# rrahn/libspm

Measured on AMD Instinct MI355X. Metric: Gbases/s scanned, Myers k<=3 |P|=100, higher is better.
Workload: dtype u32

## Files before the change

### libspm_amd/csrc/filter.hpp

```cpp
#pragma once

#include "brute.hpp"
#include "common.hpp"
#include "filter_shared.hpp"
#include "pack.hpp"
#include "hd.hpp"

namespace spm_hip
{

struct survivor
{
    uint32_t key;
    uint32_t t_lo, t_hi;
    uint32_t pad;
};
constexpr uint32_t kSurvInvalid = 0xFFFFFFFFu;

struct band_rec
{
    uint32_t slot;
    uint32_t val;
    uint32_t seg;
    uint32_t band;
// ... 785 lines not shown
                prev[4 * u + 3] = cur[u].z;
            }
            filter_words<S, NWD, HV, 4, true, KM>(P, w, prev, nv, base0 + ch * 4096, lane, lds, idx_mask);
        }
        sp += n_waves;
    }
    surv_close(P, cand_chunk_of(P, lds), lane);
}

struct verify_params
{
    const uint8_t *text;
    uint64_t text_alloc;
    uint64_t ctx_begin;
    uint64_t scan_begin;
    uint64_t scan_end;
    uint64_t pos_offset;
    const band_rec *bands;
    const unsigned long long *counters;
    uint32_t band_counter;
    uint32_t preselected;
    uint64_t band_cap;
    ulonglong2 *band_tab;
    uint32_t table_mask, band_bits;
    uint32_t runs;
    const uint8_t *surplus;
    uint32_t Bw;
    uint32_t overlap;
    uint32_t max_m;
    const uint32_t *peq32;
    uint32_t sigma;
    uint32_t nw_table;
    uint32_t max_k;
    const int32_t *m;
    const int32_t *k;
    uint32_t report_begin;
    uint32_t max_span;
    uint32_t wave_text;
    unsigned long long *seen;
    uint32_t seen_mask;
    spm_hit *hits;
    unsigned long long *hit_counter;
    uint64_t hit_cap;
    unsigned long long *overflow;
    const uint64_t *seg_offsets;
    uint64_t n_segments;
    const uint32_t *seg_owned;
};

struct resolve_params
{
    const survivor *surv;
    unsigned long long *counters;
    uint64_t surv_cap;
    const pass_entry *passes;
    const uint4 *entries;
    uint32_t key_len;
    uint32_t flank_check;
    uint32_t pieces_check;
    const uint8_t *text;
    uint64_t text_alloc;
    const uint8_t *needle_ranks;
    const uint32_t *needle_offsets;
    const uint16_t *seed_q;
    const int32_t *m, *k;
    uint64_t hay_begin, hay_end;
    const uint64_t *seg_offsets;
    uint64_t n_segments;
    uint32_t Bw, overlap, max_m;
    uint32_t band_bits;
    ulonglong2 *band_tab;
    uint32_t table_mask;
    band_rec *bands;
    uint64_t band_cap;
    const uint32_t *needle_pk;
    const uint32_t *pk_offsets;
    uint32_t exact_hits;
    uint32_t report_begin;
    uint64_t scan_begin, scan_end;
    uint64_t pos_offset;
    const uint32_t *seg_owned;
    unsigned long long *seen;
    uint32_t seen_mask;
    spm_hit *hits;
    unsigned long long *hit_counter, *overflow;
    uint64_t hit_cap;
    uint32_t *table_poison;
};

__device__ __forceinline__ unsigned long long band_value(unsigned long long stored, bool counting)
{
    return counting ? (unsigned long long)(uint32_t)(stored + 1ull) : ~stored;
}
__device__ __forceinline__ void band_release(ulonglong2 *tab, uint32_t slot)
{
    tab[slot] = make_ulonglong2(kBandEmpty, ~0ull);
}

__device__ __forceinline__ uint4 load_bytes16(const uint8_t *p)
{
    uint4 v;
    __builtin_memcpy(&v, p, 16);
    return v;
}

__device__ __forceinline__ uint4 load_bytes16_guarded(const uint8_t *base, uint64_t idx, uint64_t limit)
{
    if (idx + 16 <= limit)
        return load_bytes16(base + idx);
    uint32_t w[4] = {0xFFFFFFFFu, 0xFFFFFFFFu, 0xFFFFFFFFu, 0xFFFFFFFFu};
    for (int b = 0; b < 16; ++b)
        if (idx + b < limit)
            w[b >> 2] = (w[b >> 2] & ~(0xFFu << (8 * (b & 3)))) | ((uint32_t)base[idx + b] << (8 * (b & 3)));
    return make_uint4(w[0], w[1], w[2], w[3]);
}

__device__ __forceinline__ uint32_t diff16(const uint4 a, const uint4 b, uint32_t n)
{
    const uint32_t d[4] = {a.x ^ b.x, a.y ^ b.y, a.z ^ b.z, a.w ^ b.w};
    uint32_t r = 0;
#pragma unroll
    for (uint32_t i = 0; i < 4; ++i) {
        const uint32_t have = n > 4 * i ? n - 4 * i : 0;
        const uint32_t mask = have >= 4 ? 0xFFFFFFFFu : (have == 0 ? 0u : (1u << (8 * have)) - 1);
        r |= d[i] & mask;
    }
    return r;
}

__device__ __forceinline__ bool seed_intact(const resolve_params &P, uint64_t t, uint32_t val, uint32_t r, uint32_t q_whole,
                                            int64_t hay_b, int64_t hay_e)
{
    if (!P.needle_ranks)
        return true;
    const uint32_t pat = val >> 11, x = val & 0x7FF;
    struct
    {
        uint32_t q;
    } sp{q_whole ? q_whole : P.seed_q[pat]};
    const uint32_t o = x - r;
    const int64_t ts = (int64_t)t - (int64_t)r;
    if (ts < hay_b || ts + (int64_t)sp.q > hay_e)
        return false;
    const uint8_t *nd = P.needle_ranks + P.needle_offsets[pat] + o;
    for (uint32_t i = 0; i < sp.q; i += 16) {
        const uint32_t n = sp.q - i < 16 ? sp.q - i : 16;
        if (diff16(load_bytes16_guarded(P.text, (uint64_t)ts + i, P.text_alloc), load_bytes16(nd + i), n))
            return false;
    }
    return true;
}

constexpr uint32_t kPieceRoundsShift = 21, kPieceMissingShift = 28;

__device__ __forceinline__ bool pieces_apply(const resolve_params &P, uint64_t t, uint32_t val, uint32_t m, uint32_t k, int64_t hay_b,
                                             int64_t hay_e)
{
    if (!P.pieces_check || k == 0 || k > 7 || m < 32)
        return false;
    const int64_t d = (int64_t)t - (int64_t)(val & 0x7FF);
    return d - (int64_t)k >= hay_b && d + (int64_t)(m + k) <= hay_e;
}

__device__ __forceinline__ uint32_t pieces_visit(const resolve_params &P, uint64_t t, uint32_t val, uint32_t &rng, uint32_t m, uint32_t k)
{
    const uint32_t pat = val >> 11, x = val & 0x7FF;
    const uint32_t n_rounds = m >> 4;
    uint32_t done = (rng >> kPieceRoundsShift) & 0x7F, missing = (rng >> kPieceMissingShift) & 7;
    const bool ascending = 2 * x >= m;
    const uint32_t todo = n_rounds - done < 2 ? n_rounds - done : 2;
    const uint32_t r_lo = ascending ? done : n_rounds - done - todo;
    const uint32_t *pk = P.needle_pk + P.pk_offsets[pat] + r_lo;
    const uint32_t nw0 = pk[0], nw1 = todo == 2 ? pk[1] : 0;
    const uint64_t w0 = (uint64_t)((int64_t)t - (int64_t)x + (int64_t)(16 * r_lo) - (int64_t)k);
    const uint32_t c0 = pack16(load_bytes16_guarded(P.text, w0, P.text_alloc));
    const uint32_t c1 = pack16(load_bytes16_guarded(P.text, w0 + 16, P.text_alloc));
    const uint32_t c2 = todo == 2 ? pack16(load_bytes16_guarded(P.text, w0 + 32, P.text_alloc)) : 0;
#pragma unroll
    for (uint32_t rr = 0; rr < 2; ++rr) {
        if (rr < todo) {
            const uint32_t two = rr ? nw1 : nw0;
            const uint64_t win = rr ? ((uint64_t)c1 | ((uint64_t)c2 << 32)) : ((uint64_t)c0 | ((uint64_t)c1 << 32));
#pragma unroll
            for (uint32_t j = 0; j < 2; ++j) {
                const uint32_t piece = (two >> (16 * j)) & 0xFFFFu;
                bool found = false;
                for (uint32_t sh = 0; sh <= 2 * k; ++sh)
                    found = found || (((uint32_t)(win >> (2 * (8 * j + sh))) & 0xFFFFu) == piece);
                missing += found ? 0u : 1u;
            }
        }
    }
    if (missing > k)
        return 0;
    done += todo;
    if (done >= n_rounds)
        return 2;
    rng = (rng & ~((0x7Fu << kPieceRoundsShift) | (7u << kPieceMissingShift))) | (done << kPieceRoundsShift) |
          (missing << kPieceMissingShift);
    return 1;
}

struct text64
{
    uint64_t lo, hi;
    bool ok;
};

__device__ __forceinline__ uint32_t syms16(const text64 &W, uint32_t first)
{
    if (first >= 32)
        return (uint32_t)(W.hi >> (2 * (first - 32)));
    return (uint32_t)(W.lo >> (2 * first)) | (first ? (uint32_t)(W.hi << (2 * (32 - first)) ) : 0u);
}

__device__ __forceinline__ bool seed_sig_ok(const text64 &W, uint32_t sig, uint32_t r, uint32_t n, uint32_t H)
{
    if (n == 0)
        return true;
    const uint32_t rb = r < 16 ? r : 16;
    const uint32_t nl = rb < n ? rb : n;
    uint32_t got = nl ? syms16(W, 16 - rb) : 0u;
    if (nl < 16) {
        got &= (1u << (2 * nl)) - 1;
        got |= syms16(W, 16 + H) << (2 * nl);
    }
    const uint32_t mask = n >= 16 ? 0xFFFFFFFFu : ((1u << (2 * n)) - 1);
    return ((got ^ sig) & mask) == 0;
}

constexpr uint32_t kPairCap = 128;
struct pair_queue
{
// ... 128 lines not shown
                                                uint32_t pat, int64_t e)
{
    const unsigned long long key = ((unsigned long long)pat << 40) | (unsigned long long)e;
    uint32_t slot = (uint32_t)(mix64(key)) & seen_mask;
    for (uint32_t tries = 0; tries < 64; ++tries) {
        if (tries == 4 && __hip_atomic_load(overflow, __ATOMIC_RELAXED, __HIP_MEMORY_SCOPE_AGENT) != 0)
            return false;
        const unsigned long long old = atomicCAS(&seen[slot], ~0ull, key);
        if (old == ~0ull)
            return true;
        if (old == key)
            return false;
        slot = (slot + 1) & seen_mask;
    }
    atomicAdd(overflow, 1ull);
    return false;
}

struct resolve_wave
{
    pair_queue *Q;
    band_queue *B;
    uint32_t qn, bn;
    band_chunk C;
    uint32_t n_cand;
};

__device__ __forceinline__ void queue_sync()
{
    __builtin_amdgcn_fence(__ATOMIC_RELEASE, "wavefront");
    __builtin_amdgcn_wave_barrier();
}

__device__ __forceinline__ void check_pairs(const resolve_params &R, resolve_wave &S, uint32_t n, uint32_t lane)
{
    pair_queue &Q = *S.Q;
    band_queue &B = *S.B;
    S.qn -= n;
    const uint32_t first = S.qn;
    bool live = lane < n;
    uint64_t t = 0, seg = 0;
    uint32_t val = 0, rng = 0;
    int64_t sb = (int64_t)R.hay_begin, se = (int64_t)R.hay_end;
    if (live) {
        const uint32_t i = first + lane;
        t = ((uint64_t)Q.t_hi[i] << 32) | Q.t_lo[i];
        val = Q.val[i];
        rng = Q.rng[i];
        seg = Q.seg[i];
        if (R.seg_offsets) {
            sb = (int64_t)R.seg_offsets[seg];
            se = (int64_t)R.seg_offsets[seg + 1];
        }
    }
    queue_sync();
    bool through = live;
    const uint32_t pat = val >> 11;
    if (live && !(rng & kRngRun)) {
        if (!(rng & kSeedChecked)) {
            live = seed_intact(R, t, val, (rng >> 16) & 0x1F, (rng & kRngWhole) ? R.key_len + ((rng >> 5) & 0x1F) : 0u, sb, se);
            rng |= kSeedChecked;
        }
        through = live;
        if (live && R.pieces_check) {
            const uint32_t m = (uint32_t)R.m[pat], k = (uint32_t)R.k[pat];
            if (pieces_apply(R, t, val, m, k, sb, se)) {
                const uint32_t v = pieces_visit(R, t, val, rng, m, k);
                live = v != 0;
                through = v == 2;
            }
        }
    }
    {
        const bool back = live && !through;
        const uint64_t mm = __ballot(back);
        if (back) {
            const uint32_t q = S.qn + __popcll(mm & ((1ull << lane) - 1));
            Q.t_lo[q] = (uint32_t)t;
            Q.t_hi[q] = (uint32_t)(t >> 32);
            Q.val[q] = val;
            Q.rng[q] = rng;
            Q.seg[q] = (uint32_t)seg;
        }
        S.qn += __popcll(mm);
    }
    int64_t b_cur = 0, b_last = -1, d_lo = 0, d_hi = 0;
    if (R.exact_hits) {
        bool fresh = false;
        int64_t e = 0;
        if (live && through) {
            ++S.n_cand;
            e = (int64_t)t - (int64_t)(val & 0x7FF) + (int64_t)R.m[pat];
            int64_t own_b = (int64_t)R.scan_begin, own_e = (int64_t)R.scan_end;
            if (R.seg_offsets) {
                own_b = R.seg_owned ? sb + (int64_t)R.seg_owned[seg] : sb;
                own_e = se;
            }
            fresh = e >= own_b + 1 && e <= own_e && (!R.seen || seen_insert_raw(R.seen, R.seen_mask, R.overflow, pat, e));
        }
        const unsigned long long idx = wave_reserve_hits(R.hit_counter, fresh ? 1u : 0u);
        if (fresh && idx < R.hit_cap) {
            spm_hit h;
            h.pos = (R.report_begin ? (uint64_t)(e - (int64_t)R.m[pat]) : (uint64_t)e) + R.pos_offset;
            h.pattern = pat;
            h.score = 0;
            R.hits[idx] = h;
        }
        queue_sync();
        return;
    }
    if (live && through) {
        ++S.n_cand;
        d_hi = (int64_t)t - (int64_t)(val & 0x7FF) - sb + (int64_t)R.max_m;
        d_lo = d_hi - (int64_t)((rng & kRngRun) ? (rng & 0x7FF) : 0u);
        b_cur = d_lo / (int64_t)R.Bw;
        b_last = d_hi / (int64_t)R.Bw;
        if (R.overlap && b_cur > 0 && d_lo - b_cur * (int64_t)R.Bw <= (int64_t)R.k[pat])
            --b_cur;
        if ((uint64_t)b_last >> R.band_bits) {
            atomicAdd(&R.counters[kCntVoid], 1ull);
            b_last = b_cur - 1;
        }
    }
    for (;;) {
        const bool have = b_cur <= b_last;
        const uint64_t mm = __ballot(have);
        if (mm == 0)
            break;
        if (have) {
            const unsigned long long bkey =
                ((unsigned long long)pat << 43) | ((unsigned long long)seg << R.band_bits) | (unsigned long long)b_cur;
            const int64_t b0 = b_cur * (int64_t)R.Bw;
            const uint32_t o_lo = (uint32_t)(d_lo > b0 ? d_lo - b0 : 0);
            const uint32_t o_hi = (uint32_t)(d_hi < b0 + (int64_t)R.Bw - 1 ? d_hi - b0 : (int64_t)R.Bw - 1);
            const unsigned long long run = (o_hi - o_lo >= 63 ? ~0ull : ((1ull << (o_hi - o_lo + 1)) - 1)) << o_lo;
            const uint32_t q = S.bn + __popcll(mm & ((1ull << lane) - 1));
            B.key_lo[q] = (uint32_t)bkey;
            B.key_hi[q] = (uint32_t)(bkey >> 32);
            B.run_lo[q] = (uint32_t)run;
            B.run_hi[q] = (uint32_t)(run >> 32);
        }
        S.bn += __popcll(mm);
        queue_sync();
        if (S.bn >= 64) {
            S.bn -= 64;
            insert_bands(R, B, S.bn, 64, lane, S.C);
            queue_sync();
        }
        ++b_cur;
    }
    queue_sync();
}

__global__ __launch_bounds__(256) void resolve_kernel(const resolve_params R)
{
    __shared__ pair_queue pair_queues[4];
    __shared__ band_queue band_queues[4];
    unsigned long long n = R.counters[kCntSurvSlots];
    if (blockIdx.x == 0 && threadIdx.x == 0) {
        atomicAdd(&R.counters[kCntUnreadSurvSum], n);
        atomicMax(&R.counters[kCntUnreadSurvMax], n);
    }
    if (n > R.surv_cap)
        n = R.surv_cap;
    if (!R.exact_hits && __hip_atomic_load(R.table_poison, __ATOMIC_RELAXED, __HIP_MEMORY_SCOPE_AGENT) != 0) {
        if (blockIdx.x == 0 && threadIdx.x == 0)
            atomicAdd(&R.counters[kCntVoid], 1ull);
        return;
    }
    const uint32_t lane = threadIdx.x & 63;
    resolve_wave S;
    S.Q = &pair_queues[threadIdx.x >> 6];
    S.B = &band_queues[threadIdx.x >> 6];
    S.qn = 0;
    S.bn = 0;
    S.C.base = 0;
    S.C.used = 0;
    S.C.size = 0;
    S.C.draws = 0;
    S.n_cand = 0;
    pair_queue &Q = *S.Q;
    const uint64_t stride = (uint64_t)gridDim.x * blockDim.x;
    const uint64_t rounds = (n + stride - 1) / stride;
    for (uint64_t r = 0; r < rounds; ++r) {
        if ((r & 7u) == 7u &&
            __builtin_amdgcn_readfirstlane((uint32_t)(__hip_atomic_load(&R.counters[kCntVoid], __ATOMIC_RELAXED, __HIP_MEMORY_SCOPE_AGENT) != 0)))
            break;
        const uint64_t i = r * stride + (uint64_t)blockIdx.x * blockDim.x + threadIdx.x;
        bool probing = false;
        uint32_t key = 0;
        uint64_t t = 0, seg = 0;
        pass_entry T = R.passes[0];
        if (i < n) {
            const survivor sv = R.surv[i];
            if (sv.t_hi != kSurvInvalid) {
                probing = true;
                key = sv.key;
// ... 80 lines not shown
            OW.hi = ((uint64_t)(uint32_t)__shfl((int)(uint32_t)(W.hi >> 32), (int)owner) << 32) |
                    (uint32_t)__shfl((int)(uint32_t)W.hi, (int)owner);
            OW.ok = __shfl((int)W.ok, (int)owner) != 0;
            uint32_t val = 0, rng = 0;
            if (have) {
                const uint4 e = R.entries[o_first + (i - (o_incl - o_cnt))];
                val = e.x;
                rng = e.z;
                if (!(rng & kRngRun)) {
                    const uint32_t r0 = rng & 0x1F, ns = (rng >> 5) & 0x1F;
                    const bool whole = (rng & kRngWhole) != 0;
                    rng = (r0 << 16) | (whole ? (ns << 5) | kRngWhole : 0u);
                    if (OW.ok) {
                        if (!seed_sig_ok(OW, e.y, r0, ns, R.key_len))
                            have = false;
                        else if (whole)
                            rng |= kSeedChecked;
                    }
                }
            }
            const uint64_t mm = __ballot(have);
            if (mm != 0) {
                if (have) {
                    const uint32_t q = S.qn + __popcll(mm & ((1ull << lane) - 1));
                    Q.t_lo[q] = (uint32_t)o_t;
                    Q.t_hi[q] = (uint32_t)(o_t >> 32);
                    Q.val[q] = val;
                    Q.rng[q] = rng;
                    Q.seg[q] = o_seg;
                }
                S.qn += __popcll(mm);
                queue_sync();
                while (S.qn >= 64)
                    check_pairs(R, S, 64, lane);
            }
        }
    }
    while (S.qn != 0)
        check_pairs(R, S, S.qn < 64 ? S.qn : 64, lane);
    if (S.bn != 0)
        insert_bands(R, *S.B, 0, S.bn, lane, S.C);
    for (uint32_t q = S.C.used + lane; q < S.C.size; q += 64)
        if (S.C.base + q < R.band_cap)
            R.bands[S.C.base + q].val = kBandInvalid;
    wave_count_add(R.counters + kCntPairs, S.n_cand);
}

__device__ __forceinline__ bool seen_insert(const verify_params &P, uint32_t pat, int64_t e)
{
    return seen_insert_raw(P.seen, P.seen_mask, P.overflow, pat, e);
}

__global__ __launch_bounds__(256) void band_select_kernel(const verify_params P, band_rec *out, unsigned long long *out_count)
{
    unsigned long long n = P.counters[kCntBandSlots];
    if (n > P.band_cap)
        n = P.band_cap;
    const uint32_t lane = threadIdx.x & 63;
    const uint64_t stride = (uint64_t)gridDim.x * blockDim.x;
    const uint64_t rounds = (n + stride - 1) / stride;
    for (uint64_t r = 0; r < rounds; ++r) {
        const uint64_t i = r * stride + (uint64_t)blockIdx.x * blockDim.x + threadIdx.x;
        bool keep = false;
        band_rec c;
        c.val = kBandInvalid;
        if (i < n) {
            c = P.bands[i];
            if (c.val != kBandInvalid) {
                const uint32_t cnt = (uint32_t)band_value(P.band_tab[c.slot].y, true);
                band_release(P.band_tab, c.slot);
                keep = cnt >= (P.surplus ? (uint32_t)P.surplus[c.val >> 11] : 1u);
            }
// ... 145 lines not shown
        n = P.band_cap;
    const uint64_t stride = (uint64_t)gridDim.x * blockDim.x;
    for (uint64_t i = (uint64_t)blockIdx.x * blockDim.x + threadIdx.x; i < n; i += stride) {
        const band_rec c = bands[i];
        if (c.val != kBandInvalid)
            band_release(P.band_tab, c.slot);
    }
}

struct band_geom
{
    uint32_t pat;
    int64_t m, k;
    int64_t e_lo, e_hi;
    int64_t ws;
    int64_t dd_lo, dd_hi;
};

__device__ __forceinline__ bool decode_band(const verify_params &P, const band_rec &c, bool consume, band_geom &g)
{
    if (c.val == kBandInvalid)
        return false;
    g.pat = c.val >> 11;
    unsigned long long v = 1;
    if (!P.preselected) {
        v = band_value(P.band_tab[c.slot].y, P.overlap != 0);
        if (consume)
            band_release(P.band_tab, c.slot);
        if (c.val & kRunFollower)
            return false;
        if (P.overlap ? (uint32_t)v < (P.surplus ? (uint32_t)P.surplus[g.pat] : 1u) : v == 0)
            return false;
    }
    g.m = P.m[g.pat];
    g.k = P.k[g.pat];
    int64_t own_b = (int64_t)P.scan_begin, own_e = (int64_t)P.scan_end, hay_b = (int64_t)P.ctx_begin;
    if (P.seg_offsets) {
        const int64_t sb = (int64_t)P.seg_offsets[c.seg], se = (int64_t)P.seg_offsets[c.seg + 1];
        own_b = P.seg_owned ? sb + (int64_t)P.seg_owned[c.seg] : sb;
        own_e = se;
        hay_b = sb;
    }
    const int64_t band_base = hay_b - (int64_t)P.max_m + (int64_t)c.band * (int64_t)P.Bw;
    int64_t d = band_base;
    int64_t span = (int64_t)P.Bw - 1 + (P.overlap ? g.k + 1 : 0);
    if (!P.overlap) {
        const int lo = __ffsll((long long)v) - 1;
        int hi = 63 - __clzll((long long)v);
        if (c.val & kRunAnalysed)
            hi = (int)(((c.val >> kRunLenShift) & kRunLenMask) * P.Bw + (c.val & kRunHiMask));
        d += lo;
        span = hi - lo;
    }
    g.e_lo = d + g.m - g.k;
    g.e_hi = d + g.m + g.k + span;
    g.dd_lo = INT64_MAX;
    g.dd_hi = INT64_MIN;
    if (!P.overlap && (c.val & kRunAnalysed) && !P.seg_offsets) {
        const int64_t next_base = band_base + (int64_t)(((c.val >> kRunLenShift) & kRunLenMask) + 1) * (int64_t)P.Bw;
        g.dd_lo = (c.val & kRunTouchLeft) ? band_base + g.m + g.k : INT64_MIN;
        g.dd_hi = (c.val & kRunTouchRight) ? next_base + g.m - g.k - 1 : INT64_MAX;
    }
    if (g.e_lo < own_b + 1)
        g.e_lo = own_b + 1;
    if (g.e_hi > own_e)
        g.e_hi = own_e;
    if (g.e_lo > g.e_hi)
        return false;
// ... 389 lines not shown
```

### libspm_amd/csrc/internal.hpp

```cpp
#pragma once

#include <algorithm>
#include <chrono>
#include <cmath>
#include <cstdlib>
#include <cstring>
#include <memory>

#include "common.hpp"
#include "index_build.hpp"

using namespace spm_hip;

struct spm_patterns : spm_hip::seed_index
{
    spm_ctx *ctx = nullptr;
    int algo = 0;
    uint32_t n = 0;
    uint32_t sigma = 4;
    std::vector<uint8_t> ranks;
    std::vector<uint32_t> offsets;
    std::vector<int32_t> m, k;
    uint32_t n_groups = 0;
    uint32_t max_m = 0;
    uint32_t max_window = 0;
    uint32_t max_k = 0;
    uint32_t NW = 1;
    bool is_myers() const { return algo == SPM_ALGO_MYERS || algo == SPM_ALGO_MYERS_PREFIX; }
    void *d_arena = nullptr;
    uint32_t *d_peq = nullptr;
    uint32_t *d_peq_bot = nullptr;
    uint32_t *d_peq_verify = nullptr;
    uint32_t *d_hp0 = nullptr;
    int32_t *d_m = nullptr;
    int32_t *d_k = nullptr;
    mutable uint64_t cand_hint = 0;
    uint8_t *d_surplus = nullptr;
    uint8_t *d_ranks = nullptr;
    uint32_t *d_offsets = nullptr;
    uint32_t *d_needle_pk = nullptr;
    uint32_t *d_pk_offsets = nullptr;
    uint16_t *d_seed_q = nullptr;
    pass_entry *d_pass_tab = nullptr;
    uint4 *d_entries = nullptr;
    mutable uint64_t hit_hint = 0;
    mutable bool scanned = false;
    mutable int exact_whole = -1;
    mutable uint64_t band_hint = 0;
    spm_build_stats build{};
    mutable void *d_align = nullptr;
    mutable const uint64_t *d_al_rpeq = nullptr;
    mutable const uint32_t *d_al_rpeq_off = nullptr;
    mutable const uint8_t *d_al_ranks = nullptr;
    mutable const uint32_t *d_al_offsets = nullptr;
};

using clk = std::chrono::steady_clock;
inline float ms_since(clk::time_point t) { return std::chrono::duration<float, std::milli>(clk::now() - t).count(); }
inline bool spm_trace_on()
{
    const char *v = getenv("SPM_HIP_TRACE");
    return v && *v && *v != '0';
}


struct scan_tuning
{
    int cand_cap = 0;
    int brute_cutoff = 1;
    int verify_wave_min_words = 8;
    int span_budget = 0;
    int verify_runs = 1;
    int verify_runs_min_bands = 65536;
    int band_cap = 0;
    static scan_tuning from_env()
// ... 78 lines not shown
```

### libspm_amd/csrc/patterns.hip

```cpp
#include "internal.hpp"
#include "tables_build.hpp"

namespace
{
struct needle_upload
{
    struct item
    {
        void **dst;
        const void *src;
        size_t bytes, off;
    };
    std::vector<item> items;
    size_t total = 0;
    size_t add(void **dst, const void *src, size_t bytes, size_t zero_tail = 0)
    {
        items.push_back(item{dst, src, bytes, total});
        total += (std::max<size_t>(bytes + zero_tail, 16) + 255) & ~(size_t)255;
        return items.size() - 1;
    }
    hipError_t place(void **arena)
    {
        hipError_t e = hipMalloc(arena, std::max<size_t>(total, 256));
        if (e != hipSuccess)
// ... 76 lines not shown
        const uint32_t m = offsets[p + 1] - offsets[p];
        if (m > SPM_MAX_NEEDLE) {
            SPM_SET_ERR(ctx, "needle %u has %u symbols; limit is %u", p, m, SPM_MAX_NEEDLE);
            return SPM_E_UNSUPPORTED;
        }
        const uint32_t kk = (ps->is_myers() && k) ? k[p] : 0;
        ps->m[p] = (int32_t)m;
        ps->k[p] = (int32_t)kk;
        ps->max_m = std::max(ps->max_m, m);
        ps->max_k = std::max(ps->max_k, kk);
        ps->max_window = std::max(ps->max_window, m + kk);
    }
    ps->NW = next_pow2(std::max(1u, (ps->max_m + 31) / 32));
    const uint32_t NW = ps->NW;
    const index_tuning tune = index_tuning::from_env();
    ps->build.threads = tune.n_threads();
    needle_view nv;
    nv.algo = algo;
    nv.n = n_patterns;
    nv.sigma = sigma;
    nv.ranks = ps->ranks.data();
    nv.offsets = ps->offsets.data();
    nv.m = ps->m.data();
    nv.k = ps->k.data();
    nv.max_k = ps->max_k;
    needle_upload up;
    auto upload = [&](auto **dst, const void *src, size_t bytes) -> hipError_t {
        up.add(reinterpret_cast<void **>(dst), src, bytes);
        return hipSuccess;
    };
    double ms_upload = 0;
    long pass_tab_item = -1;
    std::vector<uint32_t> pk, pk_off;
    std::vector<uint8_t> surplus;
    auto t0 = clk::now();

    brute_tables bt;
    {
        build_brute_tables(nv, ps->n_groups, NW, sigma <= 5 || sigma == 15, tune.n_threads(), bt);
        ps->build.ms_tables = ms_since(t0);
        SPM_HIP_CHECK(ctx, upload(&ps->d_peq, bt.peq.data(), bt.peq.size() * sizeof(uint32_t)));
        if (!bt.verify.empty())
            SPM_HIP_CHECK(ctx, upload(&ps->d_peq_verify, bt.verify.data(), bt.verify.size() * sizeof(uint32_t)));
        if (!bt.bot.empty())
            SPM_HIP_CHECK(ctx, upload(&ps->d_peq_bot, bt.bot.data(), bt.bot.size() * sizeof(uint32_t)));
        if (!bt.hp0.empty())
            SPM_HIP_CHECK(ctx, upload(&ps->d_hp0, bt.hp0.data(), bt.hp0.size() * sizeof(uint32_t)));
        SPM_HIP_CHECK(ctx, upload(&ps->d_m, ps->m.data(), ps->m.size() * sizeof(int32_t)));
        SPM_HIP_CHECK(ctx, upload(&ps->d_k, ps->k.data(), ps->k.size() * sizeof(int32_t)));
    }

    if ((sigma == 4 || sigma == 5 || sigma == 15) && algo != SPM_ALGO_MYERS_PREFIX && n_patterns > 0) {
        const auto ti = clk::now();
        int rc = build_filter_index(nv, tune, *ps);
        if (rc != SPM_OK)
            return rc;
        ps->build.ms_index = ms_since(ti);
        if (!ps->fidx.empty()) {
            for (filter_index &F : ps->fidx) {
                SPM_HIP_CHECK(ctx, upload(&F.d_bitmap, F.h_image.data(), F.h_image.size() * sizeof(uint32_t)));
                SPM_HIP_CHECK(ctx, upload(&F.d_ht, F.h_ht.data(), F.h_ht.size() * sizeof(u32x4)));
                if (!F.h_buckets.empty())
                    SPM_HIP_CHECK(ctx, upload(&F.d_buckets, F.h_buckets.data(), F.h_buckets.size() * sizeof(uint16_t)));
                ps->build.keys += F.n_keys;
                for (uint32_t d = 0; d < 16; ++d)
                    ps->build.anchor_sixteenths += (F.dimer_set >> d) & 1u;
            }
            pass_tab_item = (long)up.add(reinterpret_cast<void **>(&ps->d_pass_tab), nullptr, ps->fidx.size() * sizeof(pass_entry));
            SPM_HIP_CHECK(ctx, upload(&ps->d_entries, ps->h_entries.data(), ps->h_entries.size() * sizeof(u32x4)));
            up.add(reinterpret_cast<void **>(&ps->d_ranks), ps->ranks.data(), ps->ranks.size(), 64);
            SPM_HIP_CHECK(ctx, upload(&ps->d_offsets, ps->offsets.data(), ps->offsets.size() * sizeof(uint32_t)));
            if (ps->sigma == 4) {
                pack_needles(nv, pk, pk_off, tune.n_threads());
                SPM_HIP_CHECK(ctx, upload(&ps->d_needle_pk, pk.data(), pk.size() * sizeof(uint32_t)));
                SPM_HIP_CHECK(ctx, upload(&ps->d_pk_offsets, pk_off.data(), pk_off.size() * sizeof(uint32_t)));
            }
            SPM_HIP_CHECK(ctx, upload(&ps->d_seed_q, ps->seed_q.data(), ps->seed_q.size() * sizeof(uint16_t)));
        }
        if (!ps->fidx.empty() && ps->max_k >= kMergeMinK && ps->max_k <= 1000) {
            surplus.assign(ps->m.size(), 1);
            for (uint32_t p = 0; p < ps->n; ++p)
                surplus[p] = (uint8_t)(ps->seed_n[p] - (uint32_t)ps->k[p]);
            SPM_HIP_CHECK(ctx, upload(&ps->d_surplus, surplus.data(), surplus.size()));
        }
    }
    {
        const auto tu = clk::now();
        SPM_HIP_CHECK(ctx, up.place(&ps->d_arena));
        const double ms_place = ms_since(tu);
        std::vector<pass_entry> pt;
        for (filter_index &F : ps->fidx)
            pt.push_back(pass_entry{reinterpret_cast<const uint4 *>(F.d_ht), F.ht_mask, 0});
        if (pass_tab_item >= 0)
            up.items[(size_t)pass_tab_item].src = pt.data();
        SPM_HIP_CHECK(ctx, up.stream(ctx, ps->d_arena, tune.n_threads()));
        for (filter_index &F : ps->fidx) {
            F.h_image = std::vector<uint32_t>();
            F.h_ht = std::vector<u32x4>();
            F.h_buckets = std::vector<uint16_t>();
        }
        ps->h_entries = std::vector<u32x4>();
        ps->build.bytes_device = up.total;
        ms_upload = ms_since(tu);
        if (spm_trace_on())
            fprintf(stderr, "[spm_hip] patterns_create: one allocation of %.2f MiB in %.2f ms, streamed up in %.2f ms\n",
                    up.total / 1048576.0, ms_place, ms_upload - ms_place);
    }
    ps->build.ms_upload = (float)ms_upload;
    ps->build.ms_total = ms_since(t_begin);
    ps->build.passes = (uint32_t)ps->fidx.size();
    ps->build.dense = ps->filter_dense ? 1u : 0u;
    ps->build.stride = ps->filter_stride;
    ps->build.key_len = ps->filter_key_len;
    if (spm_trace_on())
        fprintf(stderr, "[spm_hip] patterns_create: %u needles, algo %d, sigma %u -> %u pass(es)%s, %llu keys, %u/16 of the dimers; "
                        "%.2f ms (tables %.2f, index %.2f, upload %.2f; %u threads)\n",
                n_patterns, algo, sigma, ps->build.passes, ps->build.dense ? " dense" : "", (unsigned long long)ps->build.keys,
                ps->build.anchor_sixteenths, ps->build.ms_total, ps->build.ms_tables, ps->build.ms_index, ps->build.ms_upload,
// ... 169 lines not shown
```

### libspm_amd/csrc/scan_filter.hip

```cpp
#include "internal.hpp"
#include "filter.hpp"

namespace
{
template <typename K, typename... Args>
void launch(K kernel, dim3 grid, uint32_t threads, size_t lds, hipStream_t s, Args... args)
{
    hipFuncSetAttribute((const void *)kernel, hipFuncAttributeMaxDynamicSharedMemorySize, (int)lds);
    hipLaunchKernelGGL(kernel, grid, dim3(threads), lds, s, args...);
}

using filter_kernel = void (*)(filter_params);
using packed_kernel = void (*)(filter_params, const uint4 *);

template <int S, int U, bool KM>
filter_kernel sparse_kernel(uint32_t hv, uint32_t sigma)
{
    if (hv == 2 && sigma == 5)
        return seed_filter_kernel<S, U, 2, 5, KM>;
    if (hv == 2 && sigma == 15)
        return seed_filter_kernel<S, U, 2, 15, KM>;
    if (hv == 1 && sigma == 4)
        return seed_filter_kernel<S, U, 1, 4, KM>;
    if constexpr (S >= 4)
// ... 111 lines not shown
            ctx->band_slots = 0;
        }
        SPM_HIP_CHECK(ctx, hipMalloc(&ctx->d_band_tab, slots * sizeof(ulonglong2)));
        ctx->band_slots = slots;
        if (spm_trace_on())
            fprintf(stderr, "[spm_hip] band table grows to %.1f MiB: %.2f ms\n", slots * sizeof(ulonglong2) / 1048576.0, ms_since(t0));
    }
    SPM_HIP_CHECK(ctx, hipMemsetAsync(ctx->d_band_tab, 0xFF, ctx->band_slots * sizeof(ulonglong2), ctx->stream));
    SPM_HIP_CHECK(ctx, hipMemsetAsync(ctx->d_table_poison, 0, 4, ctx->stream));
    ctx->band_dirty = false;
    return SPM_OK;
}

namespace
{
static_assert(sizeof(survivor) == kSurvivorBytes && sizeof(band_rec) == kBandRecBytes, "scan_plan.hpp sizes the lists");

struct filter_run
{
    const scan_args &A;
    const retry_state &retry;
    spm_ctx *ctx;
    const spm_patterns *ps;
    spm_hits *H;
    filter_sizes Z;
    survivor *surv = nullptr;
    unsigned long long *seen = nullptr;
    band_rec *bands = nullptr;
    uint64_t *ovf = nullptr;
    const uint64_t *d_seg = nullptr;
    uint64_t n_seg = 0;
    uint32_t seg_bits = 0;
    bool exact_hits = false, skip_seen = false;

    int lay_out()
    {
        SPM_TRY(ensure_scratch(ctx, Z.surv_bytes + Z.seen_bytes + Z.band_bytes + Z.ovf_bytes));
        exact_hits = ps->max_k == 0 && !Z.overlap && ps->filter_max_range == 0 && ps->d_ranks;
        if (exact_hits && ps->exact_whole < 0) {
            bool whole = true;
            for (uint32_t p = 0; p < ps->n && whole; ++p)
                whole = ps->seed_n[p] == 1 && ps->seed_q[p] == (uint32_t)ps->m[p];
            ps->exact_whole = whole ? 1 : 0;
        }
        exact_hits = exact_hits && ps->exact_whole == 1;
        if (!exact_hits)
            SPM_TRY(ensure_band_table(ctx, Z.band_slots));
        surv = (survivor *)ctx->d_scratch;
        seen = (unsigned long long *)((uint8_t *)surv + Z.surv_bytes);
        bands = (band_rec *)((uint8_t *)seen + Z.seen_bytes);
        ovf = (uint64_t *)((uint8_t *)bands + Z.band_bytes);
        skip_seen = exact_hits && !retry.need_seen;
        if (!skip_seen)
            SPM_HIP_CHECK(ctx, hipMemsetAsync(seen, 0xFF, Z.seen_bytes, ctx->stream));
        if (!exact_hits)
            ctx->band_dirty = true;
        return SPM_OK;
    }

    int launch_passes()
    {
        filter_params P{};
        P.text = A.text->d;
        P.text_alloc = A.text->owned ? A.text->alloc : A.text->n;
        const uint64_t reach = ps->max_window;
        P.lo = A.begin >= A.ctx_begin + reach ? A.begin - reach : A.ctx_begin;
        P.hi = A.end;
        P.surv = surv;
        P.counters = H->d_count;
        P.surv_cap = Z.surv_cap;
        P.ovf_spans = ovf;
        P.ovf_cap = kOvfCap;
        for (size_t fi = 0; fi < ps->fidx.size(); ++fi) {
            const filter_index &F = ps->fidx[fi];
            P.stride = F.stride;
            P.key_len = F.key_len;
            P.key_mask = F.key_len >= 16 ? 0xFFFFFFFFu : ((1u << (2 * F.key_len)) - 1);
            P.bitmap_words = F.hash_variant == 2 ? 1024 : F.bitmap_words;
            P.lds_words = F.lds_words;
            P.chd_slot_mask = F.chd_slot_mask;
            P.chd_bucket_shift = F.chd_bucket_shift;
            P.chd_disp_off = F.chd_disp_off;
            P.n_probes = F.n_probes;
            P.bitmap = F.d_bitmap;
            P.pass = (uint32_t)fi;
            P.anchor_c = F.anchor_c;
// ... 44 lines not shown
                launch(k, dim3(grid), threads, lds, ctx->stream, Q, reinterpret_cast<const uint4 *>(A.text->d_packed));
            } else {
                const filter_kernel k = select_filter_kernel(F, ps->sigma, km);
                if (!k) {
                    SPM_SET_ERR(ctx, "internal: no filter kernel for stride %u, key length %u, sigma %u, hash variant %u, %u patterns",
                                F.stride, F.key_len, ps->sigma, F.hash_variant, F.n_pat);
                    return SPM_E_UNSUPPORTED;
                }
                launch(k, dim3(grid), threads, lds, ctx->stream, P);
            }
            SPM_HIP_CHECK(ctx, hipGetLastError());
            H->stats.main_launches++;
        }
        return SPM_OK;
    }

    template <typename Params>
    void fill_shared(Params &X) const
    {
        X.text = A.text->d;
        X.text_alloc = A.text->owned ? A.text->alloc : A.text->n;
        X.scan_begin = A.begin;
        X.scan_end = A.end;
        X.pos_offset = A.opts.pos_offset;
        X.counters = H->d_count;
        X.bands = bands;
        X.band_cap = Z.band_cap;
        X.band_tab = ctx->d_band_tab;
        X.table_mask = (uint32_t)(Z.band_slots - 1);
        X.band_bits = 43 - seg_bits;
        X.Bw = Z.Bw;
        X.overlap = Z.overlap ? 1u : 0u;
        X.max_m = ps->max_m;
        X.m = ps->d_m;
        X.k = ps->d_k;
        X.report_begin = ps->is_myers() ? 0 : 1;
        X.seen_mask = (uint32_t)(Z.seen_slots - 1);
        X.hits = H->d_hits;
        X.hit_counter = H->d_count + kCntHits;
        X.overflow = H->d_count + kCntVoid;
        X.hit_cap = H->cap;
        X.seg_offsets = d_seg;
        X.n_segments = n_seg;
        X.seg_owned = A.d_seg_owned;
    }

    int launch_resolve()
    {
        if (A.d_seg_offsets) {
            d_seg = A.d_seg_offsets;
            n_seg = A.n_segments;
        } else if (A.seg_offsets) {
            uint64_t *d = nullptr;
            SPM_HIP_CHECK(ctx, hipMalloc(&d, (A.n_segments + 1) * sizeof(uint64_t)));
            hipFree(H->d_aux[1]);
            H->d_aux[1] = d;
            SPM_HIP_CHECK(ctx, hipMemcpyAsync(d, A.seg_offsets, (A.n_segments + 1) * sizeof(uint64_t),
                                              hipMemcpyHostToDevice, ctx->stream));
            d_seg = d;
            n_seg = A.n_segments;
        }
        while (n_seg && (1ull << seg_bits) < n_seg + 1)
            ++seg_bits;
        resolve_params R{};
        fill_shared(R);
        R.surv = surv;
        R.surv_cap = Z.surv_cap;
        R.passes = ps->d_pass_tab;
        R.entries = ps->d_entries;
        R.key_len = ps->filter_key_len;
        R.needle_ranks = ps->d_ranks;
        R.needle_offsets = ps->d_offsets;
        R.seed_q = ps->d_seed_q;
        R.flank_check = (ps->sigma == 4 && !Z.overlap && R.needle_ranks) ? 1u : 0u;
        R.pieces_check = R.flank_check;
        R.hay_begin = A.ctx_begin;
        R.hay_end = A.end;
        R.needle_pk = ps->d_needle_pk;
        R.pk_offsets = ps->d_pk_offsets;
        R.exact_hits = exact_hits ? 1u : 0u;
        R.seen = skip_seen ? nullptr : seen;
        R.table_poison = ctx->d_table_poison;
        const uint64_t surv_expect = ps->cand_hint ? 2 * ps->cand_hint : Z.surv_cap;
        const uint64_t rmax = (uint64_t)ctx->n_cu * 5;
        const uint64_t per_wg = (surv_expect + 255) / 256 <= rmax ? 256 : 1024;
        const uint32_t rgrid = (uint32_t)std::min<uint64_t>(rmax, std::max<uint64_t>(ctx->n_cu / 2, (surv_expect + per_wg - 1) / per_wg));
        hipLaunchKernelGGL(resolve_kernel, dim3(rgrid), dim3(256), 0, ctx->stream, R);
        SPM_HIP_CHECK(ctx, hipGetLastError());
        return SPM_OK;
    }

    int launch_bands(bool runs)
    {
        verify_params V{};
        fill_shared(V);
        V.ctx_begin = A.ctx_begin;
        V.surplus = ps->d_surplus;
        V.peq32 = ps->d_peq_verify ? ps->d_peq_verify : ps->d_peq;
        V.sigma = ps->sigma;
        V.nw_table = ps->NW;
        V.max_k = ps->max_k;
        V.max_span = Z.max_span;
        V.seen = seen;
        V.band_counter = kCntBandSlots;
        band_rec *kept = bands + Z.band_cap;
        if (runs) {
            hipLaunchKernelGGL(band_runs_kernel, dim3(ctx->n_cu * 8), dim3(256), 0, ctx->stream, V, bands, kept, H->d_count + kCntRunHeads);
            SPM_HIP_CHECK(ctx, hipGetLastError());
            V.runs = 1;
            V.bands = kept;
            V.band_counter = kCntRunHeads;
        }
        if (Z.overlap) {
            hipLaunchKernelGGL(band_select_kernel, dim3(ctx->n_cu * 2), dim3(256), 0, ctx->stream, V, kept, H->d_count + kCntBandsSelected);
// ... 51 lines not shown
```

### libspm_amd/csrc/scan_plan.hpp

```cpp
#pragma once

#include <algorithm>
#include <cassert>
#include <cmath>
#include <cstddef>
#include <utility>
#include <vector>

#include "hd.hpp"

namespace spm_hip
{

enum scan_counter : int
{
    kCntHits = 0,
    kCntSurvSlots = 1,
    kCntVoid = 2,
    kCntBandSlots = 3,
    kCntSpanHead = 4,
    kCntPairs = 5,
    kCntSpansGaveUp = 6,
    kCntBandsVerified = 7,
    kCntUnreadSurvSum = 8,
// ... 151 lines not shown
        }
        uint64_t sidx = (uint64_t)(std::upper_bound(segs, segs + n_segments + 1, r.first) - segs);
        sidx = sidx ? sidx - 1 : 0;
        for (; sidx < n_segments && segs[sidx] < r.second; ++sidx)
            append_tiles(tab, std::max(r.first, segs[sidx]), std::min(r.second, segs[sidx + 1]), segs[sidx], F.warm, F.tile);
    }
}

struct span_plan
{
    uint32_t span_chunks = 0;
    uint32_t dynamic = 0;
};
inline span_plan plan_span(uint64_t n_chunks, uint64_t n_waves, uint32_t unit)
{
    assert(unit == 1024 || unit == 4096);
    span_plan S;
    if (unit == 4096) {
        uint64_t pspan = n_chunks / (n_waves * 8) + 1;
        pspan = std::min<uint64_t>(std::max<uint64_t>(pspan, 4), 4096);
        pspan = (pspan + 3) & ~3ull;
        S.span_chunks = (uint32_t)pspan;
        S.dynamic = pspan >= 48 ? 1u : 2u;
        return S;
    }
    uint64_t span = n_chunks / (n_waves * 32) + 1;
    if (span < 64)
        span = std::max<uint64_t>(span, std::min<uint64_t>(64, n_chunks / (n_waves * 4) + 1));
    span = std::min<uint64_t>(std::max<uint64_t>(span, 8), 4096);
    span = (span + 7) & ~7ull;
    S.span_chunks = (uint32_t)span;
    S.dynamic = span >= 192 ? 1u : 2u;
    return S;
}

constexpr uint32_t kChunkMin = 32;
constexpr size_t kSurvivorBytes = 16, kBandRecBytes = 16;

struct filter_sizes
{
    uint64_t surv_cap = 0, band_cap = 0, band_slots = 0, seen_slots = 0;
    uint32_t nwn = 1, Bw = 32, max_span = 31;
    bool use_wave = false;
    bool overlap = false;
    size_t surv_bytes = 0, seen_bytes = 0, band_bytes = 0, ovf_bytes = 0;
};

template <typename Set, typename Tune>
inline filter_sizes size_filter(const Set &ps, const Tune &tune, uint64_t symbols, uint64_t n_cu, uint64_t hit_cap, const retry_state &R)
{
    filter_sizes Z;
    const uint64_t kmax = ps.max_k;
    uint64_t est = std::max<uint64_t>(4096, 8ull * ps.n * (kmax + 1));
    est = std::max<uint64_t>(est, symbols / (ps.scanned ? 4096 : 2048));
    double chance = 0;
    for (const auto &F : ps.fidx)
        chance += (double)symbols / std::max(1u, F.stride) * (double)F.n_keys / std::pow(4.0, (double)F.key_len);
    est = std::max<uint64_t>(est, (uint64_t)(2.0 * chance));
    est = std::max<uint64_t>(est, ps.cand_hint + ps.cand_hint / 4);
    Z.surv_cap = std::min(2 * est + n_cu * 16 * kChunkMin, kSurvMax);
    if (R.cand_cap_override)
        Z.surv_cap = R.cand_cap_override;
    if (tune.cand_cap > 0)
        Z.surv_cap = (uint64_t)tune.cand_cap;
    const uint64_t band_want = std::max<uint64_t>(Z.surv_cap / 4, 2 * ps.band_hint);
    Z.band_cap = std::max<uint64_t>(band_want, 4096) * (R.band_scale ? R.band_scale : 1) + n_cu * 32 * kChunkMin;
// ... 31 lines not shown
```

Before: 6487.

## Pack per-needle metadata into one record, drain piece checks, fold seen clear into resolve

Merges m, k, pk_offset and seed_q into a single 16-byte needle_rec, so each pattern's metadata comes from one load instead of several scattered ones. In the final drain of the pair queue, the piece filter runs all remaining rounds at once in batches of eight rather than two per visit. The memset of the seen table is removed for small tables, and the resolve kernel clears it in a grid-stride loop instead. This trades a separate memset launch for extra stores inside resolve, which could race with any earlier use of the seen table in the same pass.

```diff
diff --git a/libspm_amd/csrc/filter.hpp b/libspm_amd/csrc/filter.hpp
--- a/libspm_amd/csrc/filter.hpp
+++ b/libspm_amd/csrc/filter.hpp
@@ -841,8 +841,7 @@
     uint32_t sigma;
     uint32_t nw_table;
     uint32_t max_k;
-    const int32_t *m;
-    const int32_t *k;
+    const needle_rec *needle;
     uint32_t report_begin;
     uint32_t max_span;
     uint32_t wave_text;
@@ -871,8 +870,7 @@
     uint64_t text_alloc;
     const uint8_t *needle_ranks;
     const uint32_t *needle_offsets;
-    const uint16_t *seed_q;
-    const int32_t *m, *k;
+    const needle_rec *needle;
     uint64_t hay_begin, hay_end;
     const uint64_t *seg_offsets;
     uint64_t n_segments;
@@ -883,7 +881,6 @@
     band_rec *bands;
     uint64_t band_cap;
     const uint32_t *needle_pk;
-    const uint32_t *pk_offsets;
     uint32_t exact_hits;
     uint32_t report_begin;
     uint64_t scan_begin, scan_end;
@@ -891,6 +888,8 @@
     const uint32_t *seg_owned;
     unsigned long long *seen;
     uint32_t seen_mask;
+    uint4 *seen_clear;
+    uint64_t seen_clear_n;
     spm_hit *hits;
     unsigned long long *hit_counter, *overflow;
     uint64_t hit_cap;
@@ -938,7 +937,7 @@
 }
 
 __device__ __forceinline__ bool seed_intact(const resolve_params &P, uint64_t t, uint32_t val, uint32_t r, uint32_t q_whole,
-                                            int64_t hay_b, int64_t hay_e)
+                                            const needle_rec &N, int64_t hay_b, int64_t hay_e)
 {
     if (!P.needle_ranks)
         return true;
@@ -946,7 +945,7 @@
     struct
     {
         uint32_t q;
-    } sp{q_whole ? q_whole : P.seed_q[pat]};
+    } sp{q_whole ? q_whole : N.seed_q};
     const uint32_t o = x - r;
     const int64_t ts = (int64_t)t - (int64_t)r;
     if (ts < hay_b || ts + (int64_t)sp.q > hay_e)
@@ -971,35 +970,37 @@
     return d - (int64_t)k >= hay_b && d + (int64_t)(m + k) <= hay_e;
 }
 
-__device__ __forceinline__ uint32_t pieces_visit(const resolve_params &P, uint64_t t, uint32_t val, uint32_t &rng, uint32_t m, uint32_t k)
-{
-    const uint32_t pat = val >> 11, x = val & 0x7FF;
+__device__ __forceinline__ uint32_t pieces_missing(uint32_t two, uint64_t win, uint32_t k)
+{
+    uint32_t missing = 0;
+#pragma unroll
+    for (uint32_t j = 0; j < 2; ++j) {
+        const uint32_t piece = (two >> (16 * j)) & 0xFFFFu;
+        bool found = false;
+        for (uint32_t sh = 0; sh <= 2 * k; ++sh)
+            found = found || (((uint32_t)(win >> (2 * (8 * j + sh))) & 0xFFFFu) == piece);
+        missing += found ? 0u : 1u;
+    }
+    return missing;
+}
+
+__device__ __forceinline__ uint32_t pieces_visit(const resolve_params &P, uint64_t t, uint32_t val, uint32_t &rng, const needle_rec &N)
+{
+    const uint32_t x = val & 0x7FF, m = N.m, k = N.k;
     const uint32_t n_rounds = m >> 4;
     uint32_t done = (rng >> kPieceRoundsShift) & 0x7F, missing = (rng >> kPieceMissingShift) & 7;
     const bool ascending = 2 * x >= m;
     const uint32_t todo = n_rounds - done < 2 ? n_rounds - done : 2;
     const uint32_t r_lo = ascending ? done : n_rounds - done - todo;
-    const uint32_t *pk = P.needle_pk + P.pk_offsets[pat] + r_lo;
+    const uint32_t *pk = P.needle_pk + N.pk_first + r_lo;
     const uint32_t nw0 = pk[0], nw1 = todo == 2 ? pk[1] : 0;
     const uint64_t w0 = (uint64_t)((int64_t)t - (int64_t)x + (int64_t)(16 * r_lo) - (int64_t)k);
     const uint32_t c0 = pack16(load_bytes16_guarded(P.text, w0, P.text_alloc));
     const uint32_t c1 = pack16(load_bytes16_guarded(P.text, w0 + 16, P.text_alloc));
     const uint32_t c2 = todo == 2 ? pack16(load_bytes16_guarded(P.text, w0 + 32, P.text_alloc)) : 0;
-#pragma unroll
-    for (uint32_t rr = 0; rr < 2; ++rr) {
-        if (rr < todo) {
-            const uint32_t two = rr ? nw1 : nw0;
-            const uint64_t win = rr ? ((uint64_t)c1 | ((uint64_t)c2 << 32)) : ((uint64_t)c0 | ((uint64_t)c1 << 32));
-#pragma unroll
-            for (uint32_t j = 0; j < 2; ++j) {
-                const uint32_t piece = (two >> (16 * j)) & 0xFFFFu;
-                bool found = false;
-                for (uint32_t sh = 0; sh <= 2 * k; ++sh)
-                    found = found || (((uint32_t)(win >> (2 * (8 * j + sh))) & 0xFFFFu) == piece);
-                missing += found ? 0u : 1u;
-            }
-        }
-    }
+    missing += pieces_missing(nw0, (uint64_t)c0 | ((uint64_t)c1 << 32), k);
+    if (todo == 2)
+        missing += pieces_missing(nw1, (uint64_t)c1 | ((uint64_t)c2 << 32), k);
     if (missing > k)
         return 0;
     done += todo;
@@ -1008,6 +1009,42 @@
     rng = (rng & ~((0x7Fu << kPieceRoundsShift) | (7u << kPieceMissingShift))) | (done << kPieceRoundsShift) |
           (missing << kPieceMissingShift);
     return 1;
+}
+
+constexpr uint32_t kDrainRounds = 8;
+__device__ __forceinline__ uint32_t pieces_visit_rest(const resolve_params &P, uint64_t t, uint32_t val, uint32_t rng, const needle_rec &N)
+{
+    const uint32_t x = val & 0x7FF, m = N.m, k = N.k;
+    const uint32_t n_rounds = m >> 4;
+    uint32_t done = (rng >> kPieceRoundsShift) & 0x7F, missing = (rng >> kPieceMissingShift) & 7;
+    const bool ascending = 2 * x >= m;
+    while (done < n_rounds) {
+        const uint32_t todo = n_rounds - done < kDrainRounds ? n_rounds - done : kDrainRounds;
+        const uint32_t r_lo = ascending ? done : n_rounds - done - todo;
+        const uint32_t *pk = P.needle_pk + N.pk_first + r_lo;
+        const uint64_t w0 = (uint64_t)((int64_t)t - (int64_t)x + (int64_t)(16 * r_lo) - (int64_t)k);
+        uint32_t nw[kDrainRounds], c[kDrainRounds + 1];
+#pragma unroll
+        for (uint32_t i = 0; i < kDrainRounds; ++i)
+            nw[i] = i < todo ? pk[i] : 0u;
+        if (w0 + 16 * (todo + 1) <= P.text_alloc) {
+#pragma unroll
+            for (uint32_t i = 0; i <= kDrainRounds; ++i)
+                c[i] = i <= todo ? pack16(load_bytes16(P.text + w0 + 16 * i)) : 0u;
+        } else {
+#pragma unroll
+            for (uint32_t i = 0; i <= kDrainRounds; ++i)
+                c[i] = i <= todo ? pack16(load_bytes16_guarded(P.text, w0 + 16 * i, P.text_alloc)) : 0u;
+        }
+#pragma unroll
+        for (uint32_t i = 0; i < kDrainRounds; ++i)
+            if (i < todo)
+                missing += pieces_missing(nw[i], (uint64_t)c[i] | ((uint64_t)c[i + 1] << 32), k);
+        if (missing > k)
+            return 0;
+        done += todo;
+    }
+    return 2;
 }
 
 struct text64
@@ -1202,7 +1239,7 @@
     __builtin_amdgcn_wave_barrier();
 }
 
-__device__ __forceinline__ void check_pairs(const resolve_params &R, resolve_wave &S, uint32_t n, uint32_t lane)
+__device__ __forceinline__ void check_pairs(const resolve_params &R, resolve_wave &S, uint32_t n, uint32_t lane, bool drain)
 {
     pair_queue &Q = *S.Q;
     band_queue &B = *S.B;
@@ -1226,19 +1263,19 @@
     queue_sync();
     bool through = live;
     const uint32_t pat = val >> 11;
+    needle_rec N{0, 0, 0, 0};
+    if (live)
+        N = R.needle[pat];
     if (live && !(rng & kRngRun)) {
         if (!(rng & kSeedChecked)) {
-            live = seed_intact(R, t, val, (rng >> 16) & 0x1F, (rng & kRngWhole) ? R.key_len + ((rng >> 5) & 0x1F) : 0u, sb, se);
+            live = seed_intact(R, t, val, (rng >> 16) & 0x1F, (rng & kRngWhole) ? R.key_len + ((rng >> 5) & 0x1F) : 0u, N, sb, se);
             rng |= kSeedChecked;
         }
         through = live;
-        if (live && R.pieces_check) {
-            const uint32_t m = (uint32_t)R.m[pat], k = (uint32_t)R.k[pat];
-            if (pieces_apply(R, t, val, m, k, sb, se)) {
-                const uint32_t v = pieces_visit(R, t, val, rng, m, k);
-                live = v != 0;
-                through = v == 2;
-            }
+        if (live && R.pieces_check && pieces_apply(R, t, val, N.m, N.k, sb, se)) {
+            const uint32_t v = drain ? pieces_visit_rest(R, t, val, rng, N) : pieces_visit(R, t, val, rng, N);
+            live = v != 0;
+            through = v == 2;
         }
     }
     {
@@ -1260,7 +1297,7 @@
         int64_t e = 0;
         if (live && through) {
             ++S.n_cand;
-            e = (int64_t)t - (int64_t)(val & 0x7FF) + (int64_t)R.m[pat];
+            e = (int64_t)t - (int64_t)(val & 0x7FF) + (int64_t)N.m;
             int64_t own_b = (int64_t)R.scan_begin, own_e = (int64_t)R.scan_end;
             if (R.seg_offsets) {
                 own_b = R.seg_owned ? sb + (int64_t)R.seg_owned[seg] : sb;
@@ -1271,7 +1308,7 @@
         const unsigned long long idx = wave_reserve_hits(R.hit_counter, fresh ? 1u : 0u);
         if (fresh && idx < R.hit_cap) {
             spm_hit h;
-            h.pos = (R.report_begin ? (uint64_t)(e - (int64_t)R.m[pat]) : (uint64_t)e) + R.pos_offset;
+            h.pos = (R.report_begin ? (uint64_t)(e - (int64_t)N.m) : (uint64_t)e) + R.pos_offset;
             h.pattern = pat;
             h.score = 0;
             R.hits[idx] = h;
@@ -1285,7 +1322,7 @@
         d_lo = d_hi - (int64_t)((rng & kRngRun) ? (rng & 0x7FF) : 0u);
         b_cur = d_lo / (int64_t)R.Bw;
         b_last = d_hi / (int64_t)R.Bw;
-        if (R.overlap && b_cur > 0 && d_lo - b_cur * (int64_t)R.Bw <= (int64_t)R.k[pat])
+        if (R.overlap && b_cur > 0 && d_lo - b_cur * (int64_t)R.Bw <= (int64_t)N.k)
             --b_cur;
         if ((uint64_t)b_last >> R.band_bits) {
             atomicAdd(&R.counters[kCntVoid], 1ull);
@@ -1333,6 +1370,8 @@
     }
     if (n > R.surv_cap)
         n = R.surv_cap;
+    for (uint64_t i = (uint64_t)blockIdx.x * blockDim.x + threadIdx.x; i < R.seen_clear_n; i += (uint64_t)gridDim.x * blockDim.x)
+        R.seen_clear[i] = make_uint4(0xFFFFFFFFu, 0xFFFFFFFFu, 0xFFFFFFFFu, 0xFFFFFFFFu);
     if (!R.exact_hits && __hip_atomic_load(R.table_poison, __ATOMIC_RELAXED, __HIP_MEMORY_SCOPE_AGENT) != 0) {
         if (blockIdx.x == 0 && threadIdx.x == 0)
             atomicAdd(&R.counters[kCntVoid], 1ull);
@@ -1479,12 +1518,12 @@
                 S.qn += __popcll(mm);
                 queue_sync();
                 while (S.qn >= 64)
-                    check_pairs(R, S, 64, lane);
+                    check_pairs(R, S, 64, lane, false);
             }
         }
     }
     while (S.qn != 0)
-        check_pairs(R, S, S.qn < 64 ? S.qn : 64, lane);
+        check_pairs(R, S, S.qn < 64 ? S.qn : 64, lane, true);
     if (S.bn != 0)
         insert_bands(R, *S.B, 0, S.bn, lane, S.C);
     for (uint32_t q = S.C.used + lane; q < S.C.size; q += 64)
@@ -1696,8 +1735,9 @@
         if (P.overlap ? (uint32_t)v < (P.surplus ? (uint32_t)P.surplus[g.pat] : 1u) : v == 0)
             return false;
     }
-    g.m = P.m[g.pat];
-    g.k = P.k[g.pat];
+    const needle_rec N = P.needle[g.pat];
+    g.m = N.m;
+    g.k = N.k;
     int64_t own_b = (int64_t)P.scan_begin, own_e = (int64_t)P.scan_end, hay_b = (int64_t)P.ctx_begin;
     if (P.seg_offsets) {
         const int64_t sb = (int64_t)P.seg_offsets[c.seg], se = (int64_t)P.seg_offsets[c.seg + 1];
diff --git a/libspm_amd/csrc/internal.hpp b/libspm_amd/csrc/internal.hpp
--- a/libspm_amd/csrc/internal.hpp
+++ b/libspm_amd/csrc/internal.hpp
@@ -34,13 +34,12 @@
     uint32_t *d_hp0 = nullptr;
     int32_t *d_m = nullptr;
     int32_t *d_k = nullptr;
+    needle_rec *d_needle = nullptr;
     mutable uint64_t cand_hint = 0;
     uint8_t *d_surplus = nullptr;
     uint8_t *d_ranks = nullptr;
     uint32_t *d_offsets = nullptr;
     uint32_t *d_needle_pk = nullptr;
-    uint32_t *d_pk_offsets = nullptr;
-    uint16_t *d_seed_q = nullptr;
     pass_entry *d_pass_tab = nullptr;
     uint4 *d_entries = nullptr;
     mutable uint64_t hit_hint = 0;
diff --git a/libspm_amd/csrc/patterns.hip b/libspm_amd/csrc/patterns.hip
--- a/libspm_amd/csrc/patterns.hip
+++ b/libspm_amd/csrc/patterns.hip
@@ -132,6 +132,7 @@
     double ms_upload = 0;
     long pass_tab_item = -1;
     std::vector<uint32_t> pk, pk_off;
+    std::vector<needle_rec> recs;
     std::vector<uint8_t> surplus;
     auto t0 = clk::now();
 
@@ -173,9 +174,7 @@
             if (ps->sigma == 4) {
                 pack_needles(nv, pk, pk_off, tune.n_threads());
                 SPM_HIP_CHECK(ctx, upload(&ps->d_needle_pk, pk.data(), pk.size() * sizeof(uint32_t)));
-                SPM_HIP_CHECK(ctx, upload(&ps->d_pk_offsets, pk_off.data(), pk_off.size() * sizeof(uint32_t)));
-            }
-            SPM_HIP_CHECK(ctx, upload(&ps->d_seed_q, ps->seed_q.data(), ps->seed_q.size() * sizeof(uint16_t)));
+            }
         }
         if (!ps->fidx.empty() && ps->max_k >= kMergeMinK && ps->max_k <= 1000) {
             surplus.assign(ps->m.size(), 1);
@@ -184,6 +183,10 @@
             SPM_HIP_CHECK(ctx, upload(&ps->d_surplus, surplus.data(), surplus.size()));
         }
     }
+    recs.resize(ps->m.size());
+    for (size_t p = 0; p < recs.size(); ++p)
+        recs[p] = make_needle_rec(ps->m[p], ps->k[p], p < pk_off.size() ? pk_off[p] : 0u, p < ps->seed_q.size() ? ps->seed_q[p] : 0u);
+    SPM_HIP_CHECK(ctx, upload(&ps->d_needle, recs.data(), recs.size() * sizeof(needle_rec)));
     {
         const auto tu = clk::now();
         SPM_HIP_CHECK(ctx, up.place(&ps->d_arena));
diff --git a/libspm_amd/csrc/scan_filter.hip b/libspm_amd/csrc/scan_filter.hip
--- a/libspm_amd/csrc/scan_filter.hip
+++ b/libspm_amd/csrc/scan_filter.hip
@@ -167,6 +167,7 @@
     uint64_t n_seg = 0;
     uint32_t seg_bits = 0;
     bool exact_hits = false, skip_seen = false;
+    bool resolve_clears = false;
 
     int lay_out()
     {
@@ -186,7 +187,8 @@
         bands = (band_rec *)((uint8_t *)seen + Z.seen_bytes);
         ovf = (uint64_t *)((uint8_t *)bands + Z.band_bytes);
         skip_seen = exact_hits && !retry.need_seen;
-        if (!skip_seen)
+        resolve_clears = seen_cleared_by_resolve(exact_hits, Z.seen_bytes);
+        if (!skip_seen && !resolve_clears)
             SPM_HIP_CHECK(ctx, hipMemsetAsync(seen, 0xFF, Z.seen_bytes, ctx->stream));
         if (!exact_hits)
             ctx->band_dirty = true;
@@ -297,8 +299,7 @@
         X.Bw = Z.Bw;
         X.overlap = Z.overlap ? 1u : 0u;
         X.max_m = ps->max_m;
-        X.m = ps->d_m;
-        X.k = ps->d_k;
+        X.needle = ps->d_needle;
         X.report_begin = ps->is_myers() ? 0 : 1;
         X.seen_mask = (uint32_t)(Z.seen_slots - 1);
         X.hits = H->d_hits;
@@ -336,15 +337,15 @@
         R.key_len = ps->filter_key_len;
         R.needle_ranks = ps->d_ranks;
         R.needle_offsets = ps->d_offsets;
-        R.seed_q = ps->d_seed_q;
         R.flank_check = (ps->sigma == 4 && !Z.overlap && R.needle_ranks) ? 1u : 0u;
         R.pieces_check = R.flank_check;
         R.hay_begin = A.ctx_begin;
         R.hay_end = A.end;
         R.needle_pk = ps->d_needle_pk;
-        R.pk_offsets = ps->d_pk_offsets;
         R.exact_hits = exact_hits ? 1u : 0u;
         R.seen = skip_seen ? nullptr : seen;
+        R.seen_clear = reinterpret_cast<uint4 *>(seen);
+        R.seen_clear_n = resolve_clears ? Z.seen_bytes / sizeof(uint4) : 0;
         R.table_poison = ctx->d_table_poison;
         const uint64_t surv_expect = ps->cand_hint ? 2 * ps->cand_hint : Z.surv_cap;
         const uint64_t rmax = (uint64_t)ctx->n_cu * 5;
diff --git a/libspm_amd/csrc/scan_plan.hpp b/libspm_amd/csrc/scan_plan.hpp
--- a/libspm_amd/csrc/scan_plan.hpp
+++ b/libspm_amd/csrc/scan_plan.hpp
@@ -207,6 +207,24 @@
     S.span_chunks = (uint32_t)span;
     S.dynamic = span >= 192 ? 1u : 2u;
     return S;
+}
+
+struct needle_rec
+{
+    uint32_t m, k;
+    uint32_t pk_first;
+    uint32_t seed_q;
+};
+static_assert(sizeof(needle_rec) == 16, "one 16-byte load per needle");
+SPM_HD inline needle_rec make_needle_rec(int32_t m, int32_t k, uint32_t pk_first, uint32_t seed_q)
+{
+    return needle_rec{m > 0 ? (uint32_t)m : 0u, k > 0 ? (uint32_t)k : 0u, pk_first, seed_q};
+}
+
+constexpr size_t kSeenResolveClearMax = 8u << 20;
+SPM_HD inline bool seen_cleared_by_resolve(bool exact_hits, size_t seen_bytes)
+{
+    return !exact_hits && seen_bytes <= kSeenResolveClearMax;
 }
 
 constexpr uint32_t kChunkMin = 32;
```

New measurement: 6514 (median of 5 runs). About the same (+0.4%).
